# SeanNobel/speech-decoding

Measured on AMD Instinct MI355X. Metric: train segments/sec (Gwilliams2022 208ch x 360, top-10 retrieval acc alongside), higher is better.
Workload: dtype bf16; 1 GPU; Gwilliams2022-shaped MEG: 208 ch x 360 samples, 27 subjects, F=1024, batch 256/GPU, fwd+CLIP loss+top-k+bwd+Adam (BASELINE configs[1]); global_batch=256, seq_len=360, parallelism=dp1

## Files before the change

include/sd_amd.h:

```cpp
#ifndef SD_AMD_H
#define SD_AMD_H
#include <stddef.h>
#include <stdint.h>

#ifdef __cplusplus
extern "C" {
#endif

#define SDA_ABI_VERSION 4
#define SDA_ROW_PAD 16
#define SDA_CH_ALIGN 64

enum { SDA_F32 = 0, SDA_BF16 = 1, SDA_F16 = 2 };

enum { SDA_EPI_GELU = 1,
       SDA_EPI_GLU_BWD = 4,
       SDA_EPI_GLU = 2,
       SDA_CONV_SINGLE_TILE = 4096,
       SDA_CONV_PAIR_TILES = 8192,
       SDA_CONV_ONE_PER_CU = 32768,
       SDA_CONV_FLAT_TILES = 16384,
       SDA_CONV_WIDE_TILES = 524288,
       SDA_CONV_WAVE_PRIO = 1048576,
       SDA_EPI_GELU_BWD = 65536,
// ... 80 lines not shown
                                const float* gamma, const float* beta, int C, float* partial, float* dgamma,
                                float* dbeta, int B, int T, int Cp, int dtype, void* stream);
int sda_reduce_stats(const float* partial, int nrows, float* out0, float* out1, int Cp, void* stream);
int sda_bn_gelu_backward_from_stats(const float* partial, int nrows, const void* dy, const void* x, const float* mean,
                                    const float* rstd, const float* gamma, const float* beta, int C, double count,
                                    float* dgamma, float* dbeta, float* coef, void* dx, int B, int T, int Cp, int dtype,
                                    void* stream);
int sda_bn_gelu_backward_apply(const void* dy, const void* x, const float* mean, const float* rstd,
                               const float* gamma, const float* beta, int C, const float* dgamma,
                               const float* dbeta, double count, float* coef , void* dx,
                               int B, int T, int Cp, int dtype, void* stream);
int sda_bn_gelu_backward_from_stats_dg(const float* partial, int nrows, const void* dy, const void* x, const float* mean,
                                    const float* rstd, const float* gamma, const float* beta, int C, double count,
                                    float* dgamma, float* dbeta, float* coef, void* dx, int B, int T, int Cp, int dtype,
                                    void* stream);
int sda_bn_gelu_backward_apply_dg(const void* dy, const void* x, const float* mean, const float* rstd,
                               const float* gamma, const float* beta, int C, const float* dgamma,
                               const float* dbeta, double count, float* coef , void* dx,
                               int B, int T, int Cp, int dtype, void* stream);

int sda_reduce_scratch_floats(int Cp);

int sda_zero_pad_rows(void* buf, int B, int T, int Cp, int dtype, void* stream);
int sda_fill_zero(void* p, long nbytes, void* stream);
int sda_gather_samples(const void* table, const long* idx, void* dst, int B, long sample_bytes, void* stream);
int sda_scalar_mul(const float* a, const float* b, float* out, int n, void* stream);

int sda_glu_forward(const void* x, void* y, int B, int T, int Ch, int dtype, void* stream);
int sda_glu_backward(const void* x, const void* dy, void* dx, int B, int T, int Ch, int dtype, void* stream);
int sda_gelu_backward(const void* u, const void* dz, void* du, int B, int T, int Cp, int dtype, void* stream);
int sda_reduce_scratch_rows(int B, int T);
int sda_glu_backward_colsum(const void* x, const void* dy, void* dx, float* colsum, float* scratch, int B, int T,
                            int Ch, int dtype, void* stream);
int sda_gelu_backward_colsum(const void* u, const void* dz, void* du, float* colsum, float* scratch, int B, int T,
                             int Cp, int dtype, void* stream);
int sda_glu_backward_colsum_og(const void* out, const void* gate, const void* dy, void* dx, float* colsum, float* scratch,
                               int B, int T, int Ch, int dtype, void* stream);
int sda_colsum(const void* x, float* out, float* scratch , int B, int T,
               int Cp, int dtype, void* stream);

enum { SDA_WGRAD_FLAT_ROWS = 1   };
typedef struct sda_wgrad_args {
  const void* dy;
  const void* x;
  float* g;
  void* out_e;
// ... 25 lines not shown
int sda_sa_softmax_pack(const float* a, int a_pitch, const float* mask, float* W, void* Wp, int D1, int C, int D1p,
                        int Cp, int dtype, void* stream);
int sda_sa_softmax_backward(const float* dWd, int dwd_pitch, const float* W, const float* mask, float* da,
                            int da_pitch, int D1, int C, void* stream);
int sda_sa_weights_backward(const float* dWd, const float* W, const float* mask, const float* cosT,
                            const float* sinT, float* dz, int D1, int K2, int C, int Cp, void* stream);

int sda_clip_logits_stats(const float* S, long s_pitch, const float* ysq, const float* zsq, const float* temp,
                          float* logits, float* row_max, float* row_sum, float* col_lse, float* diag , float* row_lse ,
                          int Bm, int Bn, int col0, void* stream);
int sda_clip_grad(const float* logits, const float* row_lse, const float* col_lse, const float* ysq,
                  const float* zsq, const float* temp, float inv_norm, int col0, void* G, long g_pitch,
                  float* rscale, float* cscale, float* colpart, float* scalars, int Bm, int Bn, int dtype, void* stream);
int sda_clip_grad_y(const float* logits, const float* row_lse, const float* col_lse, const float* zsq,
                    const float* zsq_all, int nz, int col0, void* Gy, long gy_pitch, int seg, int seg_pitch,
                    float* part, int Bm, int Bn, int dtype, void* stream);
int sda_clip_grad_y_finish(const float* part, int nparts, int Bg, const float* ysq, const float* zsq_all, int nz,
                           const float* temp, float inv_norm, int row0, int nrows, float* rscale_y, float* cscale_y,
                           void* stream);
int sda_clip_dz_supported(int Bm, int Bn, long row_elems, int dtype);
int sda_clip_dz(const void* G, long g_pitch, const void* Y, const void* Z, void* out, const float* cscale, const float* rscale,
                const float* out_scale, int Bm, int Bn, long row_elems, int dtype, void* stream);
int sda_clip_ranks(const float* logits, const float* diag, int32_t* cnt, int Bm, int Bn, int col0, void* stream);
int sda_clip_merge_rows(const float* all, int world, int Bg, float* lse, float* diag, void* stream);
int sda_device_count(void);
int sda_stream_create_cumask(const uint32_t* mask, int nwords, void** stream);
int sda_stream_create_priority(int priority, void** stream);
int sda_stream_destroy(void* stream);
int sda_set_cu_limit(int cus);

typedef struct sda_pgemm_args {
  const float* A;
  const float* B;
  void* C;
  int M, N, K, batch;
  long a_i, a_k, a_b;
  long b_k, b_j, b_b;
  long c_i, c_j, c_b;
  int c_dtype;
} sda_pgemm_args;
int sda_param_gemm(const sda_pgemm_args* a, void* stream);
int sda_copy3d(float* dst, long d0, long d1, long d2, const float* src, long s0, long s1, long s2, int n0, int n1, int n2,
               void* stream);
int sda_upload_words(void* dst, const void* src_host, long nwords, void* stream);

int sda_collate_rows(const float* src, float* dst, long rows, int T, int baseline_len, float clamp_lim, int clamp,
// ... 33 lines not shown
```

speech_decoding_amd/csrc/elementwise.hip:

```cpp
#include <math.h>

#include "sd_common.h"

namespace sda {

#ifndef SDA_EW_BWD_PRIO
#define SDA_EW_BWD_PRIO 3
#endif
__device__ __forceinline__ void ew_bwd_prio() {
  if constexpr (SDA_EW_BWD_PRIO > 0) __builtin_amdgcn_s_setprio(SDA_EW_BWD_PRIO);
}

struct RowWalk {
  int r, r1, step, T, b, t;
  __device__ RowWalk(int r0, int r1_, int step_, int T_) : r(r0), r1(r1_), step(step_), T(T_) {
    b = r0 / T_;
    t = r0 - b * T_;
  }
  __device__ bool valid() const { return r < r1; }
  __device__ size_t mem_row() const { return (size_t)b * rows_tp(T) + PAD + t; }
  __device__ void next() {
    r += step; t += step;
    while (t >= T) { t -= T; ++b; }
  }
// ... 858 lines not shown
  for (long i = (long)blockIdx.x * 256 + threadIdx.x; i < pad_vecs + tail_vecs; i += (long)gridDim.x * 256) {
    long v;
    if (i < pad_vecs) { const long b = i / ((long)PAD * row_vec), r = i - b * PAD * row_vec; v = b * Tp * row_vec + r; }
    else v = (long)B * Tp * row_vec + (i - pad_vecs);
    buf[v] = make_uint4(0u, 0u, 0u, 0u);
  }
}
__global__ __launch_bounds__(256) void fill_zero_kernel(uint4* __restrict__ p, long n16, int tail) {
  for (long i = (long)blockIdx.x * 256 + threadIdx.x; i < n16; i += (long)gridDim.x * 256) p[i] = make_uint4(0u, 0u, 0u, 0u);
  if (blockIdx.x == 0 && (int)threadIdx.x < tail) reinterpret_cast<unsigned char*>(p + n16)[threadIdx.x] = 0;
}
__global__ __launch_bounds__(256) void gather_samples_kernel(const uint4* __restrict__ table, const long* __restrict__ idx,
                                                             uint4* __restrict__ dst, long vecs) {
  const uint4* __restrict__ src = table + (size_t)idx[blockIdx.y] * vecs;
  uint4* __restrict__ out = dst + (size_t)blockIdx.y * vecs;
  long i = (long)blockIdx.x * 256 + threadIdx.x;
  const long step = (long)gridDim.x * 256;
  for (; i + 3 * step < vecs; i += 4 * step) {
    const uint4 a = src[i], b = src[i + step], c = src[i + 2 * step], d = src[i + 3 * step];
    out[i] = a; out[i + step] = b; out[i + 2 * step] = c; out[i + 3 * step] = d;
  }
  for (; i < vecs; i += step) out[i] = src[i];
}
__global__ void scalar_mul_kernel(const float* __restrict__ a, const float* __restrict__ b, float* __restrict__ out, int n) {
  const int i = blockIdx.x * blockDim.x + threadIdx.x;
  if (i < n) out[i] = a[i] * b[0];
}
}

extern "C" int sda_zero_pad_rows(void* buf, int B, int T, int Cp, int dtype, void* stream) {
  if (!buf || B < 1 || T < 1 || Cp % 64) { set_error("zero_pad_rows: bad arguments"); return -1; }
  const int row_vec = Cp * (dtype == SDA_F32 ? 4 : 2) / 16;
  const long n = ((long)B * PAD + (rows_alloc(B, T) - (long)B * rows_tp(T))) * row_vec;
  const long blocks = (n + 255) / 256;
  hipLaunchKernelGGL(zero_pad_rows_kernel, dim3((unsigned)(blocks < 1024 ? blocks : 1024)), dim3(256), 0, (hipStream_t)stream,
                     (uint4*)buf, B, rows_tp(T), rows_alloc(B, T), row_vec);
  return check_launch("zero_pad_rows");
}

extern "C" int sda_fill_zero(void* p, long nbytes, void* stream) {
  if (!p || nbytes < 1 || (reinterpret_cast<uintptr_t>(p) & 15)) { set_error("fill_zero: null, empty or unaligned buffer"); return -1; }
  const long n16 = nbytes / 16;
  const long blocks = (n16 + 255) / 256;
  hipLaunchKernelGGL(fill_zero_kernel, dim3((unsigned)(blocks < 1 ? 1 : (blocks > 2048 ? 2048 : blocks))), dim3(256), 0, (hipStream_t)stream,
                     (uint4*)p, n16, (int)(nbytes - n16 * 16));
  return check_launch("fill_zero");
}

extern "C" int sda_gather_samples(const void* table, const long* idx, void* dst, int B, long sample_bytes, void* stream) {
  if (!table || !idx || !dst || B < 1 || sample_bytes < 16 || sample_bytes % 16 || (reinterpret_cast<uintptr_t>(table) & 15) ||
      (reinterpret_cast<uintptr_t>(dst) & 15)) {
    set_error("gather_samples: bad arguments (samples are whole 16-byte vectors)"); return -1;
  }
  const long vecs = sample_bytes / 16;
  long bx = (vecs + 256 * 4 - 1) / (256 * 4);
  const long want = (8L * launch_cus() + B - 1) / B;
  if (bx > want) bx = want;
  if (bx < 1) bx = 1;
  hipLaunchKernelGGL(gather_samples_kernel, dim3((unsigned)bx, (unsigned)B), dim3(256), 0, (hipStream_t)stream,
                     (const uint4*)table, idx, (uint4*)dst, vecs);
// ... 409 lines not shown
```

speech_decoding_amd/csrc/sa_loss.hip:

```cpp
#include "sd_common.h"

namespace sda {

__device__ inline float block_sum(float v, float* sh) {
  v = wave_sum(v);
  __syncthreads();
  if ((threadIdx.x & 63) == 0) sh[threadIdx.x >> 6] = v;
  __syncthreads();
  return sh[0] + sh[1] + sh[2] + sh[3];
}
__device__ inline float block_max(float v, float* sh) {
  v = wave_max(v);
  __syncthreads();
  if ((threadIdx.x & 63) == 0) sh[threadIdx.x >> 6] = v;
  __syncthreads();
  return fmaxf(fmaxf(sh[0], sh[1]), fmaxf(sh[2], sh[3]));
}

constexpr int SA_R = 8;
constexpr int SA_MC = 128;

__global__ __launch_bounds__(256) void sa_fwd_partial_kernel(const float* __restrict__ z, const float* __restrict__ cos_t,
                                                             const float* __restrict__ sin_t, float* __restrict__ part,
                                                             int D1, int K2, int C) {
// ... 258 lines not shown
  pd[threadIdx.x] = dt;
  __syncthreads();
  if (threadIdx.x != 0) return;
  l = 0.0; dt = 0.0;
  for (int k = 0; k < 64; ++k) { l += pl[k]; dt += pd[k]; }
  scalars[0] = (float)(l * (double)inv_norm);
  scalars[1] = (float)dt;
}

__global__ __launch_bounds__(256) void clip_ranks_kernel(const float* __restrict__ logits, const float* __restrict__ diag,
                                                         int32_t* __restrict__ cnt, int Bm, int Bn, int col0) {
  __shared__ float sh[4];
  const int i = blockIdx.x, tid = threadIdx.x;
  const float d = diag[i];
  float c = 0.f;
  for (int j = tid; j < Bn; j += 256) {
    const float l = logits[(size_t)i * Bn + j];
    if (l > d || (l == d && col0 + j < i)) c += 1.f;
  }
  c = block_sum(c, sh);
  if (tid == 0) cnt[i] = (int32_t)(c + 0.5f);
}

}

using namespace sda;

extern "C" int sda_sa_scratch_floats(int D1, int K2, int C) { return ((K2 + SA_MC - 1) / SA_MC) * D1 * C; }

extern "C" int sda_sa_weights_forward(const float* z, const float* cos_t, const float* sin_t, const float* mask, float* W,
                                      void* Wp, float* scratch, int D1, int K2, int C, int D1p, int Cp, int dtype, void* stream) {
  if (!z || !cos_t || !sin_t || !W || !Wp || !scratch || C > 512 || C > Cp || D1 > D1p) { set_error("sa_weights_forward: bad arguments (C <= 512)"); return -1; }
  hipStream_t st = (hipStream_t)stream;
  const int nchunk = (K2 + SA_MC - 1) / SA_MC;
  hipLaunchKernelGGL(sa_fwd_partial_kernel, dim3((D1 + SA_R - 1) / SA_R, nchunk), dim3(256), 0, st, z, cos_t, sin_t, scratch, D1, K2, C);
  if (dtype == SDA_F32)
    hipLaunchKernelGGL(sa_fwd_final_kernel<float>, dim3(D1p), dim3(256), 0, st, scratch, nchunk, C, mask, W, (float*)Wp, D1, C, Cp);
  else if (dtype == SDA_BF16)
    hipLaunchKernelGGL(sa_fwd_final_kernel<uint16_t>, dim3(D1p), dim3(256), 0, st, scratch, nchunk, C, mask, W, (uint16_t*)Wp, D1, C, Cp);
  else if (dtype == SDA_F16)
    hipLaunchKernelGGL(sa_fwd_final_kernel<half_t>, dim3(D1p), dim3(256), 0, st, scratch, nchunk, C, mask, W, (half_t*)Wp, D1, C, Cp);
  else { set_error("sa_weights_forward: unknown dtype"); return -1; }
  return check_launch("sa_weights_forward");
}

extern "C" int sda_sa_softmax_pack(const float* a, int a_pitch, const float* mask, float* W, void* Wp, int D1, int C,
                                   int D1p, int Cp, int dtype, void* stream) {
  if (!a || !W || !Wp || C > 512 || C > Cp || D1 > D1p || a_pitch < C) { set_error("sa_softmax_pack: bad arguments (C <= 512)"); return -1; }
  hipStream_t st = (hipStream_t)stream;
// ... 121 lines not shown
```

speech_decoding_amd/engine.py:

```python
from __future__ import annotations

from dataclasses import dataclass, field
from typing import Dict, List, Optional

import ast
import os

import numpy as np
import torch

from . import lib as L
from . import ops


def block_dilations(k: int):
    return 2 ** ((2 * k) % 5), 2 ** ((2 * k + 1) % 5), 2


@dataclass
class EncoderDims:
    C: int
    S: int
    D1: int
    D2: int
# ... 673 lines not shown
@dataclass
class ClipCtx:
    Bm: int
    Bn: int
    col0: int
    G: torch.Tensor
    rscale: torch.Tensor
    Yt: torch.Tensor
    Zt: torch.Tensor
    row_elems: int
    dtemp: torch.Tensor
    cscale: Optional[torch.Tensor] = None
    logits: Optional[torch.Tensor] = None
    row_lse: Optional[torch.Tensor] = None
    col_lse: Optional[torch.Tensor] = None
    ysq: Optional[torch.Tensor] = None
    zsq: Optional[torch.Tensor] = None
    temp: Optional[torch.Tensor] = None
    inv_norm: float = 0.0


def clip_forward(Yt: torch.Tensor, Zt: torch.Tensor, temp: torch.Tensor, *, Bm: int, Bn: int, T: int, col0: int = 0,
                 reduction: str = "mean", B_global: Optional[int] = None, dist_group=None, want_grad: bool = True,
                 ysq: Optional[torch.Tensor] = None):
    st = clip_block_stats(Yt, Zt, temp, Bm=Bm, Bn=Bn, T=T, col0=col0, ysq=ysq)
    if dist_group is None:
        row_lse, diag = st.row_lse, st.diag
    else:
        from .distributed import merge_row_softmax_stats
        row_lse, diag = merge_row_softmax_stats(st.row_max, st.row_sum, dist_group, diag=st.diag)
    return clip_block_finish(st, row_lse, diag, reduction=reduction, B_global=B_global)


@dataclass
class ClipBlockStats:
    Yt: torch.Tensor
    Zt: torch.Tensor
    temp: torch.Tensor
    Bm: int
    Bn: int
    col0: int
    row_elems: int
    ysq: torch.Tensor
    zsq: torch.Tensor
    logits: torch.Tensor
    row_max: torch.Tensor
    row_sum: torch.Tensor
    col_lse: torch.Tensor
    diag: torch.Tensor
    row_lse: torch.Tensor


def clip_block_stats(Yt, Zt, temp, *, Bm: int, Bn: int, T: int, col0: int = 0, ysq=None) -> ClipBlockStats:
    Fp = Zt.shape[1]
# ... 32 lines not shown
```

speech_decoding_amd/lib.py:

```python
from __future__ import annotations

import ctypes as C
import os

_HERE = os.path.dirname(os.path.abspath(__file__))
LIB_PATH = os.path.join(_HERE, "libsdamd.so")

ABI_VERSION = 4
F32, BF16, F16 = 0, 1, 2
ROW_PAD = 16
CH_ALIGN = 64
EPI_GELU, EPI_GLU, EPI_GLU_BWD = 1, 2, 4
EPI_GELU_BWD, EPI_ROW_SUMSQ, EPI_BN_STORE_DG = 65536, 131072, 262144
CONV_SINGLE_TILE, CONV_PAIR_TILES, CONV_FLAT_TILES, CONV_ONE_PER_CU = 4096, 8192, 16384, 32768
CONV_WAVE_PRIO = 1048576
CONV_WIDE_TILES = 524288
WGRAD_FLAT_ROWS = 1

vp, i32, i64, f32, f64 = C.c_void_p, C.c_int, C.c_long, C.c_float, C.c_double


class ConvArgs(C.Structure):
    _fields_ = [("x", vp), ("w", vp), ("bias", vp), ("res", vp), ("y", vp), ("y_pre", vp), ("widx", vp),
                ("stats", vp), ("partial", vp), ("bn_x", vp), ("bn_coef", vp), ("glu_out", vp), ("glu_gate", vp),
# ... 86 lines not shown
    "sda_sa_scratch_floats": (i32, [i32, i32, i32]),
    "sda_sa_softmax_pack": (i32, [vp, i32, vp, vp, vp, i32, i32, i32, i32, i32, vp]),
    "sda_sa_softmax_backward": (i32, [vp, i32, vp, vp, vp, i32, i32, i32, vp]),
    "sda_sa_weights_backward": (i32, [vp, vp, vp, vp, vp, vp, i32, i32, i32, i32, vp]),
    "sda_clip_logits_stats": (i32, [vp, i64, vp, vp, vp, vp, vp, vp, vp, vp, vp, i32, i32, i32, vp]),
    "sda_clip_grad": (i32, [vp, vp, vp, vp, vp, vp, f32, i32, vp, i64, vp, vp, vp, vp, i32, i32, i32, vp]),
    "sda_clip_grad_y": (i32, [vp, vp, vp, vp, vp, i32, i32, vp, i64, i32, i32, vp, i32, i32, i32, vp]),
    "sda_clip_grad_y_finish": (i32, [vp, i32, i32, vp, vp, i32, vp, f32, i32, i32, vp, vp, vp]),
    "sda_collate_rows": (i32, [vp, vp, i64, i32, i32, f32, i32, vp]),
    "sda_collate_windows": (i32, [vp, vp, vp, i32, i32, i32, i32, f32, i32, vp]),
    "sda_clip_ranks": (i32, [vp, vp, vp, i32, i32, i32, vp]),
    "sda_clip_dz_supported": (i32, [i32, i32, i64, i32]),
    "sda_clip_dz": (i32, [vp, i64, vp, vp, vp, vp, vp, vp, i32, i32, i64, i32, vp]),
    "sda_param_gemm": (i32, [C.POINTER(PgemmArgs), vp]),
    "sda_zero_pad_rows": (i32, [vp, i32, i32, i32, i32, vp]),
    "sda_scalar_mul": (i32, [vp, vp, vp, i32, vp]),
    "sda_fill_zero": (i32, [vp, i64, vp]),
    "sda_gather_samples": (i32, [vp, vp, vp, i32, i64, vp]),
    "sda_clip_merge_rows": (i32, [vp, i32, i32, vp, vp, vp]),
    "sda_copy3d": (i32, [vp, i64, i64, i64, vp, i64, i64, i64, i32, i32, i32, vp]),
    "sda_mse_forward": (i32, [vp, i32, i32, vp, i32, i32, i32, i32, i32, i32, vp, vp, vp]),
    "sda_mse_backward": (i32, [vp, i32, i32, vp, i32, i32, i32, i32, i32, i32, vp, vp, vp, vp]),
    "sda_input_grad": (i32, [vp, i64, vp, vp, i32, i32, i32, i32, i32, i32, i32, vp, i32, vp]),
}
MSE_PARTIALS = 2048

_lib = None


class SdaError(RuntimeError):
    pass


def load():
    global _lib
    if _lib is not None:
        return _lib
    if not os.path.exists(LIB_PATH):
        raise SdaError(
            f"{LIB_PATH} not found: the HIP extension is required (no CPU fallback). "
            "Build it with `python -c 'import __graft_entry__ as g; g.build()'` "
            "or `make -C speech_decoding_amd/csrc`.")
    lib = C.CDLL(LIB_PATH)
    for name, (res, args) in SIGNATURES.items():
        fn = getattr(lib, name)
        fn.restype = res
# ... 24 lines not shown
```

speech_decoding_amd/loss.py:

```python
from __future__ import annotations

from typing import Optional

import torch
import torch.nn as nn

from . import lib as L
from . import ops
from . import engine as E

import weakref

_rank_cache = []


class LossState:

    def __init__(self):
        self.rings = {}
        self.prefetched = []
        self.ring_depth = 2
        self.emulated = {}

    def drain(self):
# ... 170 lines not shown
        Yt, ysq, Bm, col0, Bg, works, slot = gather_speech_rows(Yt_local, B, T, group, async_op=True, state=state, slot=slot)
    state.prefetched.clear()
    state.prefetched.append((weakref.ref(Y), dtype, Yt, ysq, Bm, col0, Bg, works, done, slot))


def _take_prefetched(state: LossState, Y, dtype):
    for wy, dt, Yt, ysq, Bm, col0, Bg, works, done, slot in state.prefetched:
        if wy() is Y and dt == dtype:
            state.prefetched.clear()
            if done is not None:
                torch.cuda.current_stream(Yt.device).wait_event(done)
            for work in works:
                work.wait()
            return Yt, ysq, Bm, col0, Bg, slot
    return None


_RECYCLED = ("CLIPLoss.backward: the packed {what} rows of this forward were recycled by later forwards of the same CLIPLoss "
             "(more than `ring_depth` forwards before this backward); raise loss_func._state.ring_depth or call backward earlier")


class _ClipFn(torch.autograd.Function):
    @staticmethod
    def forward(ctx, module: "CLIPLoss", Y, Z, temp):
        import torch.distributed as dist
        B, F, T = Z.shape
        dtype = Z.dtype if Z.dtype in ops.COMPUTE_DTYPES else torch.float32
        Zt = as_rows(Z, B, F, T, dtype, "y (brain embeddings)")
        group = _dist_group() if module.global_negatives else None
        state = module._state
        want_y = ctx.needs_input_grad[1]
        y_rows = False
        if want_y:
            y_rows = _rows_base(Y, B, F, T, dtype) is not None
            if not y_rows and not Y.is_cuda:
                raise L.SdaError("CLIPLoss: x (speech embeddings) must live on the MI355X device (there is no CPU path)")
            if not y_rows and Y.dtype not in ops.COMPUTE_DTYPES:
                raise L.SdaError(f"CLIPLoss: a speech embedding that requires a gradient must be fp32, bf16 or fp16, got {Y.dtype}")
            if group is not None and dist.get_world_size(group) == 1:
                from .distributed import emulated_world
                if emulated_world() > 1:
                    raise L.SdaError("CLIPLoss: the emulated world (stand-in rows for the other ranks) has no gradient for the "
                                     "speech embeddings; detach x or run real ranks")
        pre = _take_prefetched(state, Y, dtype)
        if pre is not None:
            Yt, ysq, Bm, col0, Bg, slot = pre
        else:
            Yt_local, slot = as_rows(Y, B, F, T, dtype, "x (speech embeddings)", ring_key="loss.Y", state=state, want_slot=True)
            Yt, ysq, Bm, col0, Bg, _, slot = gather_speech_rows(Yt_local, B, T, group, state=state, slot=slot)
        loss, logits, cnt, cctx = E.clip_forward(Yt, Zt, temp.detach(), Bm=Bm, Bn=B, T=T, col0=col0,
                                                 reduction=module.reduction, B_global=Bg, dist_group=group, ysq=ysq)
        ctx.z_gather = None
        if want_y and group is not None:
            Zall, zsq_all, _, _, _, works, zslot = gather_speech_rows(Zt, B, T, group, async_op=True, state=state,
                                                                      ring_key="loss.Zall", sq=cctx.zsq)
            ctx.z_gather = (Zall, zsq_all, works, zslot)
        if group is not None:
            both = torch.cat([cnt.to(torch.float32), loss.reshape(1)])
            dist.all_reduce(both, group=group)
            cnt, loss = both[:-1].round().to(torch.int32), both[-1:]
        ctx.cctx, ctx.shape, ctx.dtype, ctx.group = cctx, (B, F, T), dtype, group
        ctx.set_materialize_grads(False)
        ctx.y_slot = slot
        ctx.z_requires_grad = Z.requires_grad
        ctx.y_requires_grad, ctx.y_rows, ctx.y_dtype = want_y, y_rows, Y.dtype
        _cache_ranks(Y, Z, cnt[col0: col0 + B])
        ctx.mark_non_differentiable(logits)
        return loss.reshape(()), logits

    @staticmethod
    def backward(ctx, dloss, _dlogits):
        c = ctx.cctx
        B, F, T = ctx.shape
        dZ = dY = None
        if dloss is None:
            return None, None, None, None
        scale = dloss.to(torch.float32)
        if (ctx.z_requires_grad or ctx.y_requires_grad) and ctx.y_slot is not None and not ctx.y_slot.valid():
            raise L.SdaError(_RECYCLED.format(what="speech"))
        if ctx.z_requires_grad:
            dZt = ops.new_rows_uninit(B, T, c.Zt.shape[1], ctx.dtype, c.Zt.device)
            E.clip_backward(c, dZt, scale.reshape(1).contiguous())
            dZ = ops.rows_view(dZt, B, F, T)
        if ctx.y_requires_grad:
            dYt = _clip_dy(ctx, scale.reshape(1).contiguous())
            dY = ops.rows_view(dYt, B, F, T) if ctx.y_rows else ops.unpack_rows_typed(dYt, B, F, T, ctx.y_dtype)
        dtemp = ops.scalar_mul(c.dtemp, scale.reshape(1))
        return None, dY, dZ, dtemp


def _clip_dy(ctx, scale: torch.Tensor) -> torch.Tensor:
    c = ctx.cctx
    B, F, T = ctx.shape
    dYt = ops.new_rows_uninit(B, T, c.Yt.shape[1], ctx.dtype, c.Yt.device)
    if ctx.group is None:
        E.clip_backward_y(c, dYt, scale)
        return dYt
    import torch.distributed as dist
    from .distributed import side_group
    world, rank = dist.get_world_size(ctx.group), dist.get_rank(ctx.group)
    Zall, zsq_all, works, zslot = ctx.z_gather
    for work in works:
        work.wait()
    if not zslot.valid():
        raise L.SdaError(_RECYCLED.format(what="brain"))
    Bg, sp = c.Bm, L.pad_channels(B)
    Gy, part = ops.clip_grad_y(c.logits, c.row_lse, c.col_lse, c.zsq, zsq_all, c.col0, ctx.dtype, seg=B, seg_pitch=sp,
                               groups=world)
    Gall = torch.empty((Bg + 1, world * sp), dtype=ctx.dtype, device=Gy.device)
    ops.fill_zero_(Gall[Bg])
    pall = torch.empty((world * part.shape[0], Bg), dtype=torch.float32, device=Gy.device)
# ... 13 lines not shown
        L.load()
        self.reduction = str(args.reduction)
        if self.reduction not in ("mean", "sum"):
            raise ValueError("reduction must be 'mean' or 'sum'")
        self.temp = nn.Parameter(torch.tensor([float(args.init_temperature)]))
        self.global_negatives = True
        self.last_logits: Optional[torch.Tensor] = None
        self._state = LossState()

    def prefetch(self, x: torch.Tensor, compute_dtype=torch.float32):
        prefetch_speech(x, compute_dtype, self.global_negatives, state=self._state)

    def drain(self):
        self._state.drain()

    def release_buffers(self):
        self._state.clear()

    def forward(self, x, y, fast=True, return_logits=False):
        batch_size = x.size(0)
        assert batch_size > 1, "Batch size must be greater than 1."
        if not fast:
            zero = torch.zeros(1, dtype=torch.float32, device=self.temp.device)
            loss, logits = _ClipFn.apply(self, x, y, zero)
            self.last_logits = logits
            return (logits.t(), loss) if return_logits else loss
        loss, logits = _ClipFn.apply(self, x, y, self.temp)
        self.last_logits = logits
        if return_logits:
            return logits, loss
        return loss


@torch.no_grad()
def retrieval_ranks(Y: torch.Tensor, Z: torch.Tensor, global_candidates: bool = True) -> torch.Tensor:
    hit = _cached_ranks(Y, Z)
    if hit is not None:
        return hit
    B, F, T = Z.shape
    dtype = Z.dtype if Z.dtype in ops.COMPUTE_DTYPES else torch.float32
    Zt = as_rows(Z, B, F, T, dtype, "Z")
    Yt = as_rows(Y, B, F, T, dtype, "Y")
    temp = torch.zeros(1, dtype=torch.float32, device=Zt.device)
    group = _dist_group() if global_candidates else None
    Yt, ysq, Bm, col0, Bg, _, _ = gather_speech_rows(Yt, B, T, group)
    _, _, cnt, _ = E.clip_forward(Yt, Zt, temp, Bm=Bm, Bn=B, T=T, col0=col0, B_global=Bg, dist_group=group, ysq=ysq)
    if group is not None:
        import torch.distributed as dist
        dist.all_reduce(cnt, group=group)
    return cnt[col0: col0 + B]
# ... 75 lines not shown
```

speech_decoding_amd/ops.py:

```python
from __future__ import annotations

import ctypes as C
import os
from typing import Optional

import numpy as np
import torch

from . import lib as L

_DT = {torch.float32: L.F32, torch.bfloat16: L.BF16, torch.float16: L.F16}
COMPUTE_DTYPES = tuple(_DT)


def dt_code(dtype: torch.dtype) -> int:
    try:
        return _DT[dtype]
    except KeyError:
        raise L.SdaError(f"unsupported compute dtype {dtype}; use torch.float32, torch.bfloat16 or torch.float16")


def _p(t: Optional[torch.Tensor]):
    return None if t is None else t.data_ptr()

# ... 103 lines not shown
        raise L.SdaError("fill_zero_: a contiguous tensor")
    if t.numel():
        L.check(L.load().sda_fill_zero(t.data_ptr(), t.numel() * t.element_size(), _st()), "fill_zero")
    return t


def gather_samples(table: torch.Tensor, idx: torch.Tensor, B: int, T: int) -> torch.Tensor:
    _need_cuda(table, idx)
    if idx.dtype != torch.int64 or idx.numel() != B:
        raise L.SdaError("gather_samples: idx must hold B int64 indices")
    Cp = table.shape[1]
    out = new_rows_uninit(B, T, Cp, table.dtype, table.device)
    L.check(L.load().sda_gather_samples(_p(table), _p(idx), _p(out), B, L.rows_tp(T) * Cp * table.element_size(), _st()), "gather_samples")
    return out


def clip_merge_rows(allp: torch.Tensor):
    world, k, Bg = allp.shape
    if k != 3 or allp.dtype != torch.float32 or not allp.is_contiguous():
        raise L.SdaError("clip_merge_rows: a contiguous fp32 (world, 3, B_global) table")
    out = torch.empty((2, Bg), dtype=torch.float32, device=allp.device)
    L.check(L.load().sda_clip_merge_rows(_p(allp), world, Bg, _p(out[0]), _p(out[1]), _st()), "clip_merge_rows")
    return out[0], out[1]


def scalar_mul(a: torch.Tensor, b: torch.Tensor) -> torch.Tensor:
    out = torch.empty_like(a)
    L.check(L.load().sda_scalar_mul(_p(a), _p(b), _p(out), a.numel(), _st()), "scalar_mul")
    return out


def rows_view(buf: torch.Tensor, B: int, C: int, T: int) -> torch.Tensor:
    Tp, Cp = L.rows_tp(T), buf.shape[1]
    return buf.as_strided((B, C, T), (Tp * Cp, 1, Cp), L.ROW_PAD * Cp)


def pack_rows(src: torch.Tensor, dst: torch.Tensor, ones_channel: Optional[int] = None):
    _need_cuda(src, dst)
    B, Cc, T = src.shape
    src = src.contiguous().float()
    if ones_channel is None:
        L.check(L.load().sda_pack_rows(_p(src), _p(dst), B, Cc, T, dst.shape[1], dt_code(dst.dtype), _st()), "pack_rows")
    else:
        L.check(L.load().sda_pack_rows_ones(_p(src), _p(dst), B, Cc, T, dst.shape[1], ones_channel, dt_code(dst.dtype), _st()),
                "pack_rows_ones")

# ... 302 lines not shown
        cin, cout = alg_dims if alg_dims is not None else (x.shape[1], y.shape[1])
        e0, e1 = torch.cuda.Event(enable_timing=True), torch.cuda.Event(enable_timing=True)
        e0.record()
        L.check(L.load().sda_conv_gemm(C.byref(a), _st()), "conv_gemm")
        e1.record()
        TIMER.records.append((("conv_gemm", str(x.dtype).replace("torch.", ""), conv_tile_co(Cout_p, KS, stats is not None), KS),
                              2.0 * B * T * KS * cin * cout, e0, e1))
        return y
    L.check(L.load().sda_conv_gemm(C.byref(a), _st()), "conv_gemm")
    return y


def n_t_tiles(T: int) -> int:
    return (T + 127) // 128


def conv_stats_rows(B: int, T: int, KS: int, Cout_p: int, flags: int = 0) -> int:
    return L.load().sda_conv_stats_rows(B, T, KS, Cout_p, flags)


SIM_GEMM_TILES256 = os.environ.get("SDA_SIM_GEMM", "1") != "0"


def matmul_nt_splitk(xm: torch.Tensor, wm: torch.Tensor, M: int, N: int, K: int, pitch: int) -> torch.Tensor:
    Np = L.pad_channels(N)
    if SIM_GEMM_TILES256 and K <= pitch:
        ks = L.load().sda_sim_gemm_ksplit(M, N, K, dt_code(xm.dtype))
        if ks > 0:
            partial = torch.empty((ks, M, Np), dtype=torch.float32, device=xm.device)
            L.check(L.load().sda_sim_gemm(_p(xm), _p(wm), _p(partial), M, N, Np, K, pitch, ks, dt_code(xm.dtype), _st()), "sim_gemm")
            if ks == 1:
                return partial[0]
            out = torch.empty((M, Np), dtype=torch.float32, device=xm.device)
            L.check(L.load().sda_reduce_slabs(_p(partial), _p(out), ks, M * Np, _st()), "reduce_slabs")
            return out
    slab = 32 if xm.dtype == torch.float32 else 64
    nslab = K // slab
    tile_co = 160 if Np % 160 == 0 else (128 if Np % 128 == 0 else 64)
    tiles = ((M + 127) // 128) * (Np // tile_co)
    ksplit = max(1, min(nslab, (512 + tiles - 1) // tiles))
    if nslab <= 64:
        ksplit = min(ksplit, 16)
    partial = torch.empty((ksplit, M, Np), dtype=torch.float32, device=xm.device)
    a = L.ConvArgs()
    a.x, a.w, a.bias, a.res, a.y, a.y_pre, a.widx, a.stats = _p(xm), _p(wm), None, None, None, None, None, None
    a.partial = _p(partial)
    a.B, a.T, a.Cin_p, a.Cout_p, a.KS, a.dil = 1, M, K, Np, 1, 0
    a.x_pitch, a.w_pitch, a.x_row0, a.x_sample_rows, a.x_rows_limit = pitch, pitch, 0, 0, M
    a.w_rows_limit, a.ksplit, a.flags, a.dtype = N, ksplit, 0, dt_code(xm.dtype)
    L.check(L.load().sda_conv_gemm(C.byref(a), _st()), "conv_gemm(split-K)")
    if ksplit == 1:
        return partial[0]
    out = torch.empty((M, Np), dtype=torch.float32, device=xm.device)
    L.check(L.load().sda_reduce_slabs(_p(partial), _p(out), ksplit, M * Np, _st()), "reduce_slabs")
    return out


def bn_finalize(partial, ntiles, count, gamma, beta, running_mean, running_var, Cp, training, eps=1e-5, momentum=0.1,
                want_bwd_coef=False, batches_tracked=None):
    if batches_tracked is not None and (batches_tracked.dtype != torch.int64 or not batches_tracked.is_cuda):
        raise L.SdaError("bn_finalize: batches_tracked must be an int64 device tensor")
    dev = gamma.device
    buf = torch.empty((8 if want_bwd_coef else 4, Cp), dtype=torch.float32, device=dev)
    mean, rstd, scale, shift = buf[0], buf[1], buf[2], buf[3]
    coef = buf[4:] if want_bwd_coef else None
    L.check(L.load().sda_bn_finalize(_p(partial), ntiles, float(count), _p(gamma), _p(beta), eps, momentum,
                                     _p(running_mean), _p(running_var), _p(mean), _p(rstd), _p(scale), _p(shift),
                                     _p(coef), gamma.numel(), Cp, int(training), _p(batches_tracked), _st()), "bn_finalize")
    return (mean, rstd, scale, shift, coef) if want_bwd_coef else (mean, rstd, scale, shift)


def bn_gelu_forward(x, y, scale, shift, B, T):
    L.check(L.load().sda_bn_gelu_forward(_p(x), _p(y), _p(scale), _p(shift), B, T, x.shape[1], dt_code(x.dtype), _st()),
# ... 233 lines not shown
    st3 = torch.empty((3, Bm), dtype=torch.float32, device=dev)
    row_max, row_sum, diag = st3[0], st3[1], st3[2]
    col_lse = torch.empty(Bn, dtype=torch.float32, device=dev)
    row_lse = torch.empty(Bm, dtype=torch.float32, device=dev)
    L.check(L.load().sda_clip_logits_stats(_p(S), S.shape[1], _p(ysq), _p(zsq), _p(temp), _p(logits), _p(row_max), _p(row_sum),
                                           _p(col_lse), _p(diag), _p(row_lse), Bm, Bn, col0, _st()), "clip_logits_stats")
    return logits, row_max, row_sum, col_lse, diag, row_lse


def clip_grad(logits, row_lse, col_lse, ysq, zsq, temp, inv_norm, col0, dtype):
    Bm, Bn = logits.shape
    dev = logits.device
    G = torch.empty((Bm + 1, L.pad_channels(Bn)), dtype=dtype, device=dev)
    rscale = torch.empty(Bn, dtype=torch.float32, device=dev)
    cscale = torch.empty(Bn, dtype=torch.float32, device=dev)
    colpart = torch.empty(2 * Bn, dtype=torch.float32, device=dev)
    scalars = torch.empty(2, dtype=torch.float32, device=dev)
    L.check(L.load().sda_clip_grad(_p(logits), _p(row_lse), _p(col_lse), _p(ysq), _p(zsq), _p(temp), float(inv_norm), col0,
                                   _p(G), G.shape[1], _p(rscale), _p(cscale), _p(colpart), _p(scalars), Bm, Bn, dt_code(dtype), _st()),
            "clip_grad")
    return G, rscale, cscale, scalars


def clip_grad_y(logits, row_lse, col_lse, zsq, zsq_all, col0, dtype, *, seg=None, seg_pitch=None, groups=1):
    Bm, Bn = logits.shape
    seg = Bm if seg is None else seg
    seg_pitch = L.pad_channels(seg) if seg_pitch is None else seg_pitch
    dev = logits.device
    Gy = torch.empty((Bn + 1, groups * seg_pitch), dtype=dtype, device=dev)
    part = torch.empty(((Bn + 63) // 64, Bm), dtype=torch.float32, device=dev)
    L.check(L.load().sda_clip_grad_y(_p(logits), _p(row_lse), _p(col_lse), _p(zsq), _p(zsq_all), zsq_all.numel(), col0, _p(Gy),
                                     Gy.shape[1], seg, seg_pitch, _p(part), Bm, Bn, dt_code(dtype), _st()), "clip_grad_y")
    return Gy, part


def clip_grad_y_finish(part, ysq, zsq_all, temp, inv_norm, row0, nrows):
    nparts, Bg = part.shape
    rscale = torch.empty(nrows, dtype=torch.float32, device=part.device)
    cscale = torch.empty(nrows, dtype=torch.float32, device=part.device)
    L.check(L.load().sda_clip_grad_y_finish(_p(part), nparts, Bg, _p(ysq), _p(zsq_all), zsq_all.numel(), _p(temp), float(inv_norm),
                                            row0, nrows, _p(rscale), _p(cscale), _st()), "clip_grad_y_finish")
    return rscale, cscale


def clip_ranks(logits, diag, col0):
    Bm, Bn = logits.shape
# ... 76 lines not shown
```

Before: 38070 segments/s.

## Fuse CLIP split-K reduction, logits stats, ranks and grad into two kernels

The single-GPU CLIP forward path now keeps the split-K similarity partials unreduced. A row kernel sums the slabs while computing logits, row softmax stats and rank counts, and a column kernel computes column LSE, the gradient matrix, scales and the final loss scalars, using a last-block atomic reduction. The backward pass also folds the dtemp scalar multiply into the zero-padding kernel for dZ. The aim is fewer small kernel launches in the loss section. The cost is a grid-wide atomic counter and a limit of 256 rows for the fused path.

```diff
diff --git a/include/sd_amd.h b/include/sd_amd.h
--- a/include/sd_amd.h
+++ b/include/sd_amd.h
@@ -126,6 +126,8 @@
 int sda_reduce_scratch_floats(int Cp);
 
 int sda_zero_pad_rows(void* buf, int B, int T, int Cp, int dtype, void* stream);
+int sda_zero_pad_rows_scaled(void* buf, int B, int T, int Cp, int dtype, const float* a, const float* b, float* out, int n,
+                             void* stream);
 int sda_fill_zero(void* p, long nbytes, void* stream);
 int sda_gather_samples(const void* table, const long* idx, void* dst, int B, long sample_bytes, void* stream);
 int sda_scalar_mul(const float* a, const float* b, float* out, int n, void* stream);
@@ -197,6 +199,11 @@
 int sda_clip_dz(const void* G, long g_pitch, const void* Y, const void* Z, void* out, const float* cscale, const float* rscale,
                 const float* out_scale, int Bm, int Bn, long row_elems, int dtype, void* stream);
 int sda_clip_ranks(const float* logits, const float* diag, int32_t* cnt, int Bm, int Bn, int col0, void* stream);
+int sda_clip_stats_fused_max_rows(void);
+int sda_clip_stats_fused(const float* slabs, int nslabs, long slab_elems, long s_pitch, const float* ysq, const float* zsq,
+                         const float* temp, const float* dloss, float inv_norm, float* logits, float* row_max, float* row_sum,
+                         float* row_lse, float* col_lse, float* diag, void* G, long g_pitch, float* rscale, float* cscale,
+                         float* colpart, float* scalars, int32_t* cnt, unsigned* counter, int B, int dtype, void* stream);
 int sda_clip_merge_rows(const float* all, int world, int Bg, float* lse, float* diag, void* stream);
 int sda_device_count(void);
 int sda_stream_create_cumask(const uint32_t* mask, int nwords, void** stream);
diff --git a/speech_decoding_amd/csrc/elementwise.hip b/speech_decoding_amd/csrc/elementwise.hip
--- a/speech_decoding_amd/csrc/elementwise.hip
+++ b/speech_decoding_amd/csrc/elementwise.hip
@@ -904,6 +904,19 @@
   }
   for (; i < vecs; i += step) out[i] = src[i];
 }
+__global__ __launch_bounds__(256) void zero_pad_rows_scaled_kernel(uint4* __restrict__ buf, int B, int Tp, long rows_alloc, int row_vec,
+                                                                   const float* __restrict__ a, const float* __restrict__ b,
+                                                                   float* __restrict__ out, int n) {
+  if (blockIdx.x == 0)
+    for (int i = threadIdx.x; i < n; i += 256) out[i] = a[i] * b[0];
+  const long pad_vecs = (long)B * PAD * row_vec, tail_vecs = (rows_alloc - (long)B * Tp) * row_vec;
+  for (long i = (long)blockIdx.x * 256 + threadIdx.x; i < pad_vecs + tail_vecs; i += (long)gridDim.x * 256) {
+    long v;
+    if (i < pad_vecs) { const long bb = i / ((long)PAD * row_vec), r = i - bb * PAD * row_vec; v = bb * Tp * row_vec + r; }
+    else v = (long)B * Tp * row_vec + (i - pad_vecs);
+    buf[v] = make_uint4(0u, 0u, 0u, 0u);
+  }
+}
 __global__ void scalar_mul_kernel(const float* __restrict__ a, const float* __restrict__ b, float* __restrict__ out, int n) {
   const int i = blockIdx.x * blockDim.x + threadIdx.x;
   if (i < n) out[i] = a[i] * b[0];
@@ -918,6 +931,17 @@
   hipLaunchKernelGGL(zero_pad_rows_kernel, dim3((unsigned)(blocks < 1024 ? blocks : 1024)), dim3(256), 0, (hipStream_t)stream,
                      (uint4*)buf, B, rows_tp(T), rows_alloc(B, T), row_vec);
   return check_launch("zero_pad_rows");
+}
+
+extern "C" int sda_zero_pad_rows_scaled(void* buf, int B, int T, int Cp, int dtype, const float* a, const float* b, float* out, int n,
+                                        void* stream) {
+  if (!buf || B < 1 || T < 1 || Cp % 64 || !a || !b || !out || n < 1) { set_error("zero_pad_rows_scaled: bad arguments"); return -1; }
+  const int row_vec = Cp * (dtype == SDA_F32 ? 4 : 2) / 16;
+  const long nv = ((long)B * PAD + (rows_alloc(B, T) - (long)B * rows_tp(T))) * row_vec;
+  const long blocks = (nv + 255) / 256;
+  hipLaunchKernelGGL(zero_pad_rows_scaled_kernel, dim3((unsigned)(blocks < 1024 ? blocks : 1024)), dim3(256), 0, (hipStream_t)stream,
+                     (uint4*)buf, B, rows_tp(T), rows_alloc(B, T), row_vec, a, b, out, n);
+  return check_launch("zero_pad_rows_scaled");
 }
 
 extern "C" int sda_fill_zero(void* p, long nbytes, void* stream) {
diff --git a/speech_decoding_amd/csrc/sa_loss.hip b/speech_decoding_amd/csrc/sa_loss.hip
--- a/speech_decoding_amd/csrc/sa_loss.hip
+++ b/speech_decoding_amd/csrc/sa_loss.hip
@@ -304,9 +304,145 @@
   if (tid == 0) cnt[i] = (int32_t)(c + 0.5f);
 }
 
+__global__ __launch_bounds__(256) void clip_stats_rows_kernel(const float* __restrict__ slabs, int nslabs, long slab_elems,
+                                                              long s_pitch, const float* __restrict__ ysq,
+                                                              const float* __restrict__ zsq, const float* __restrict__ temp,
+                                                              float* __restrict__ logits, float* __restrict__ row_max,
+                                                              float* __restrict__ row_sum, float* __restrict__ diag,
+                                                              float* __restrict__ row_lse, int32_t* __restrict__ cnt,
+                                                              unsigned* __restrict__ counter, int B) {
+  __shared__ float sh[4];
+  __shared__ float dsh;
+  const int i = blockIdx.x, tid = threadIdx.x;
+  const bool valid = tid < B;
+  if (i == 0 && tid == 0) *counter = 0u;
+  const float alpha = expf(temp[0]);
+  const float ri = alpha / sqrtf(ysq[i]);
+  float l = -INFINITY;
+  if (valid) {
+    const float* __restrict__ src = slabs + (size_t)i * s_pitch + tid;
+    float s = 0.f;
+    int k = 0;
+    for (; k + 8 <= nslabs; k += 8) {
+      float v[8];
+#pragma unroll
+      for (int j = 0; j < 8; ++j) v[j] = src[(size_t)(k + j) * slab_elems];
+#pragma unroll
+      for (int j = 0; j < 8; ++j) s += v[j];
+    }
+    for (; k < nslabs; ++k) s += src[(size_t)k * slab_elems];
+    l = s * ri / sqrtf(zsq[tid]);
+    logits[(size_t)i * B + tid] = l;
+    if (tid == i) { diag[i] = l; dsh = l; }
+  }
+  const float mx = block_max(l, sh);
+  const float sum = block_sum(valid ? expf(l - mx) : 0.f, sh);
+  if (tid == 0) { row_max[i] = mx; row_sum[i] = sum; row_lse[i] = mx + logf(sum); }
+  const float d = dsh;
+  float c = 0.f;
+  if (valid && (l > d || (l == d && tid < i))) c += 1.f;
+  c = block_sum(c, sh);
+  if (tid == 0) cnt[i] = (int32_t)(c + 0.5f);
+}
+
+template <typename E>
+__global__ __launch_bounds__(256) void clip_stats_cols_kernel(const float* __restrict__ logits, const float* __restrict__ row_lse,
+                                                              const float* __restrict__ ysq, const float* __restrict__ zsq,
+                                                              const float* __restrict__ temp, const float* __restrict__ dloss,
+                                                              float inv_norm, float* __restrict__ col_lse, E* __restrict__ G,
+                                                              long g_pitch, float* __restrict__ rscale, float* __restrict__ cscale,
+                                                              float* colpart, float* __restrict__ scalars, unsigned* counter, int B) {
+  __shared__ float sh[4];
+  __shared__ double pl[64], pd[64];
+  __shared__ int last;
+  const int j = blockIdx.x, tid = threadIdx.x;
+  const bool valid = tid < B;
+  if (tid == 0) Elem<E>::st(G + (size_t)B * g_pitch + j, 0.f);
+  if (j >= B) {
+    if (valid) Elem<E>::st(G + (size_t)tid * g_pitch + j, 0.f);
+  } else {
+    const float l = valid ? logits[(size_t)tid * B + j] : -INFINITY;
+    const float mx = block_max(l, sh);
+    const float sum = block_sum(valid ? expf(l - mx) : 0.f, sh);
+    const float cl = mx + logf(sum);
+    const float ymax = sqrtf(block_max(valid ? fmaxf(0.f, ysq[tid]) : 0.f, sh));
+    const float alpha = expf(temp[0]);
+    float dl = 0.f;
+    if (valid) {
+      float d = expf(l - row_lse[tid]) + expf(l - cl);
+      if (tid == j) d -= 2.f;
+      dl += d * l;
+      Elem<E>::st(G + (size_t)tid * g_pitch + j, d * (ymax / sqrtf(ysq[tid])));
+    }
+    dl = block_sum(dl, sh) * inv_norm;
+    if (tid == 0) {
+      const float ljj = logits[(size_t)j * B + j];
+      col_lse[j] = cl;
+      rscale[j] = dl / zsq[j];
+      cscale[j] = inv_norm * alpha / (ymax * sqrtf(zsq[j]));
+      colpart[j * 2 + 0] = (row_lse[j] - ljj) + (cl - ljj);
+      colpart[j * 2 + 1] = dl;
+    }
+  }
+  if (tid == 0) {
+    __threadfence();
+    const unsigned t = __hip_atomic_fetch_add(counter, 1u, __ATOMIC_ACQ_REL, __HIP_MEMORY_SCOPE_AGENT);
+    last = (t == gridDim.x - 1);
+  }
+  __syncthreads();
+  if (!last) return;
+  __threadfence();
+  if (tid < 64) {
+    double ls = 0.0, dt = 0.0;
+    for (int k = tid; k < B; k += 64) {
+      ls += (double)__hip_atomic_load(colpart + k * 2, __ATOMIC_RELAXED, __HIP_MEMORY_SCOPE_AGENT);
+      dt += (double)__hip_atomic_load(colpart + k * 2 + 1, __ATOMIC_RELAXED, __HIP_MEMORY_SCOPE_AGENT);
+    }
+    pl[tid] = ls;
+    pd[tid] = dt;
+  }
+  __syncthreads();
+  if (tid != 0) return;
+  double ls = 0.0, dt = 0.0;
+  for (int k = 0; k < 64; ++k) { ls += pl[k]; dt += pd[k]; }
+  scalars[0] = (float)(ls * (double)inv_norm);
+  scalars[1] = (float)dt;
+  if (dloss) scalars[2] = (float)dt * dloss[0];
+}
+
 }
 
 using namespace sda;
+
+extern "C" int sda_clip_stats_fused_max_rows(void) { return 256; }
+
+extern "C" int sda_clip_stats_fused(const float* slabs, int nslabs, long slab_elems, long s_pitch, const float* ysq,
+                                    const float* zsq, const float* temp, const float* dloss, float inv_norm, float* logits,
+                                    float* row_max, float* row_sum, float* row_lse, float* col_lse, float* diag, void* G,
+                                    long g_pitch, float* rscale, float* cscale, float* colpart, float* scalars, int32_t* cnt,
+                                    unsigned* counter, int B, int dtype, void* stream) {
+  if (!slabs || !ysq || !zsq || !temp || !logits || !row_max || !row_sum || !row_lse || !col_lse || !diag || !G || !rscale ||
+      !cscale || !colpart || !scalars || !cnt || !counter) { set_error("clip_stats_fused: null argument"); return -1; }
+  if (B < 1 || B > 256 || nslabs < 1 || s_pitch < B || slab_elems < (long)(B - 1) * s_pitch + B || g_pitch < B || g_pitch > 65535) {
+    set_error("clip_stats_fused: 1 <= B <= 256 rows and columns, slabs of at least B rows of s_pitch >= B floats, g_pitch >= B");
+    return -1;
+  }
+  hipStream_t st = (hipStream_t)stream;
+  hipLaunchKernelGGL(clip_stats_rows_kernel, dim3(B), dim3(256), 0, st, slabs, nslabs, slab_elems, s_pitch, ysq, zsq, temp, logits,
+                     row_max, row_sum, diag, row_lse, cnt, counter, B);
+  const dim3 grid((unsigned)g_pitch);
+  if (dtype == SDA_F32)
+    hipLaunchKernelGGL(clip_stats_cols_kernel<float>, grid, dim3(256), 0, st, logits, row_lse, ysq, zsq, temp, dloss, inv_norm, col_lse,
+                       (float*)G, g_pitch, rscale, cscale, colpart, scalars, counter, B);
+  else if (dtype == SDA_BF16)
+    hipLaunchKernelGGL(clip_stats_cols_kernel<uint16_t>, grid, dim3(256), 0, st, logits, row_lse, ysq, zsq, temp, dloss, inv_norm, col_lse,
+                       (uint16_t*)G, g_pitch, rscale, cscale, colpart, scalars, counter, B);
+  else if (dtype == SDA_F16)
+    hipLaunchKernelGGL(clip_stats_cols_kernel<half_t>, grid, dim3(256), 0, st, logits, row_lse, ysq, zsq, temp, dloss, inv_norm, col_lse,
+                       (half_t*)G, g_pitch, rscale, cscale, colpart, scalars, counter, B);
+  else { set_error("clip_stats_fused: unknown dtype"); return -1; }
+  return check_launch("clip_stats_fused");
+}
 
 extern "C" int sda_sa_scratch_floats(int D1, int K2, int C) { return ((K2 + SA_MC - 1) / SA_MC) * D1 * C; }
 
diff --git a/speech_decoding_amd/engine.py b/speech_decoding_amd/engine.py
--- a/speech_decoding_amd/engine.py
+++ b/speech_decoding_amd/engine.py
@@ -719,7 +719,9 @@
 
 def clip_forward(Yt: torch.Tensor, Zt: torch.Tensor, temp: torch.Tensor, *, Bm: int, Bn: int, T: int, col0: int = 0,
                  reduction: str = "mean", B_global: Optional[int] = None, dist_group=None, want_grad: bool = True,
-                 ysq: Optional[torch.Tensor] = None):
+                 ysq: Optional[torch.Tensor] = None, fused: bool = False):
+    if fused and dist_group is None and Bm == Bn and col0 == 0 and Bm <= ops.clip_stats_fused_max_rows():
+        return _clip_forward_fused(Yt, Zt, temp, B=Bm, T=T, reduction=reduction, B_global=B_global, ysq=ysq)
     st = clip_block_stats(Yt, Zt, temp, Bm=Bm, Bn=Bn, T=T, col0=col0, ysq=ysq)
     if dist_group is None:
         row_lse, diag = st.row_lse, st.diag
@@ -727,6 +729,23 @@
         from .distributed import merge_row_softmax_stats
         row_lse, diag = merge_row_softmax_stats(st.row_max, st.row_sum, dist_group, diag=st.diag)
     return clip_block_finish(st, row_lse, diag, reduction=reduction, B_global=B_global)
+
+
+def _clip_forward_fused(Yt, Zt, temp, *, B: int, T: int, reduction: str, B_global: Optional[int], ysq):
+    row_elems = L.rows_tp(T) * Zt.shape[1]
+    if ysq is None:
+        ysq = ops.rows_sumsq(Yt, B, row_elems, row_elems)
+    zsq = ops.ROW_NORMS.get(Zt, B)
+    if zsq is None:
+        zsq = ops.rows_sumsq(Zt, B, row_elems, row_elems)
+    slabs = ops.matmul_nt_splitk(Yt, Zt, B, B, row_elems, row_elems, reduce=False)
+    Bg = B_global if B_global is not None else B
+    inv_norm = 1.0 / (2.0 * Bg) if reduction == "mean" else 0.5
+    logits, _, _, col_lse, _, row_lse, G, rscale, cscale, scalars, cnt = ops.clip_stats_fused(slabs, ysq, zsq, temp, inv_norm,
+                                                                                              Yt.dtype, B)
+    ctx = ClipCtx(Bm=B, Bn=B, col0=0, G=G, rscale=rscale, Yt=Yt, Zt=Zt, row_elems=row_elems, dtemp=scalars[1:2],
+                  cscale=cscale, logits=logits, row_lse=row_lse, col_lse=col_lse, ysq=ysq, zsq=zsq, temp=temp, inv_norm=inv_norm)
+    return scalars[0:1], logits, cnt, ctx
 
 
 @dataclass
diff --git a/speech_decoding_amd/lib.py b/speech_decoding_amd/lib.py
--- a/speech_decoding_amd/lib.py
+++ b/speech_decoding_amd/lib.py
@@ -132,6 +132,10 @@
     "sda_mse_forward": (i32, [vp, i32, i32, vp, i32, i32, i32, i32, i32, i32, vp, vp, vp]),
     "sda_mse_backward": (i32, [vp, i32, i32, vp, i32, i32, i32, i32, i32, i32, vp, vp, vp, vp]),
     "sda_input_grad": (i32, [vp, i64, vp, vp, i32, i32, i32, i32, i32, i32, i32, vp, i32, vp]),
+    "sda_clip_stats_fused_max_rows": (i32, []),
+    "sda_clip_stats_fused": (i32, [vp, i32, i64, i64, vp, vp, vp, vp, f32, vp, vp, vp, vp, vp, vp, vp, i64, vp, vp, vp, vp, vp, vp,
+                                   i32, i32, vp]),
+    "sda_zero_pad_rows_scaled": (i32, [vp, i32, i32, i32, i32, vp, vp, vp, i32, vp]),
 }
 MSE_PARTIALS = 2048
 
diff --git a/speech_decoding_amd/loss.py b/speech_decoding_amd/loss.py
--- a/speech_decoding_amd/loss.py
+++ b/speech_decoding_amd/loss.py
@@ -216,7 +216,7 @@
 
 class _ClipFn(torch.autograd.Function):
     @staticmethod
-    def forward(ctx, module: "CLIPLoss", Y, Z, temp):
+    def forward(ctx, module: "CLIPLoss", Y, Z, temp, fast):
         import torch.distributed as dist
         B, F, T = Z.shape
         dtype = Z.dtype if Z.dtype in ops.COMPUTE_DTYPES else torch.float32
@@ -243,7 +243,8 @@
             Yt_local, slot = as_rows(Y, B, F, T, dtype, "x (speech embeddings)", ring_key="loss.Y", state=state, want_slot=True)
             Yt, ysq, Bm, col0, Bg, _, slot = gather_speech_rows(Yt_local, B, T, group, state=state, slot=slot)
         loss, logits, cnt, cctx = E.clip_forward(Yt, Zt, temp.detach(), Bm=Bm, Bn=B, T=T, col0=col0,
-                                                 reduction=module.reduction, B_global=Bg, dist_group=group, ysq=ysq)
+                                                 reduction=module.reduction, B_global=Bg, dist_group=group, ysq=ysq,
+                                                 fused=fast and group is None and not want_y)
         ctx.z_gather = None
         if want_y and group is not None:
             Zall, zsq_all, _, _, _, works, zslot = gather_speech_rows(Zt, B, T, group, async_op=True, state=state,
@@ -268,19 +269,21 @@
         B, F, T = ctx.shape
         dZ = dY = None
         if dloss is None:
-            return None, None, None, None
+            return None, None, None, None, None
         scale = dloss.to(torch.float32)
         if (ctx.z_requires_grad or ctx.y_requires_grad) and ctx.y_slot is not None and not ctx.y_slot.valid():
             raise L.SdaError(_RECYCLED.format(what="speech"))
         if ctx.z_requires_grad:
-            dZt = ops.new_rows_uninit(B, T, c.Zt.shape[1], ctx.dtype, c.Zt.device)
+            dZt, dtemp = ops.zero_pad_rows_scaled(torch.empty((L.rows_alloc(B, T), c.Zt.shape[1]), dtype=ctx.dtype, device=c.Zt.device),
+                                                  B, T, c.dtemp, scale.reshape(1))
             E.clip_backward(c, dZt, scale.reshape(1).contiguous())
             dZ = ops.rows_view(dZt, B, F, T)
         if ctx.y_requires_grad:
             dYt = _clip_dy(ctx, scale.reshape(1).contiguous())
             dY = ops.rows_view(dYt, B, F, T) if ctx.y_rows else ops.unpack_rows_typed(dYt, B, F, T, ctx.y_dtype)
-        dtemp = ops.scalar_mul(c.dtemp, scale.reshape(1))
-        return None, dY, dZ, dtemp
+        if not ctx.z_requires_grad:
+            dtemp = ops.scalar_mul(c.dtemp, scale.reshape(1))
+        return None, dY, dZ, dtemp, None
 
 
 def _clip_dy(ctx, scale: torch.Tensor) -> torch.Tensor:
@@ -340,10 +343,10 @@
         assert batch_size > 1, "Batch size must be greater than 1."
         if not fast:
             zero = torch.zeros(1, dtype=torch.float32, device=self.temp.device)
-            loss, logits = _ClipFn.apply(self, x, y, zero)
+            loss, logits = _ClipFn.apply(self, x, y, zero, False)
             self.last_logits = logits
             return (logits.t(), loss) if return_logits else loss
-        loss, logits = _ClipFn.apply(self, x, y, self.temp)
+        loss, logits = _ClipFn.apply(self, x, y, self.temp, True)
         self.last_logits = logits
         if return_logits:
             return logits, loss
diff --git a/speech_decoding_amd/ops.py b/speech_decoding_amd/ops.py
--- a/speech_decoding_amd/ops.py
+++ b/speech_decoding_amd/ops.py
@@ -149,6 +149,13 @@
     out = torch.empty((2, Bg), dtype=torch.float32, device=allp.device)
     L.check(L.load().sda_clip_merge_rows(_p(allp), world, Bg, _p(out[0]), _p(out[1]), _st()), "clip_merge_rows")
     return out[0], out[1]
+
+
+def zero_pad_rows_scaled(buf: torch.Tensor, B: int, T: int, a: torch.Tensor, b: torch.Tensor):
+    out = torch.empty_like(a)
+    L.check(L.load().sda_zero_pad_rows_scaled(_p(buf), B, T, buf.shape[1], dt_code(buf.dtype), _p(a), _p(b), _p(out), a.numel(), _st()),
+            "zero_pad_rows_scaled")
+    return buf, out
 
 
 def scalar_mul(a: torch.Tensor, b: torch.Tensor) -> torch.Tensor:
@@ -497,13 +504,15 @@
 SIM_GEMM_TILES256 = os.environ.get("SDA_SIM_GEMM", "1") != "0"
 
 
-def matmul_nt_splitk(xm: torch.Tensor, wm: torch.Tensor, M: int, N: int, K: int, pitch: int) -> torch.Tensor:
+def matmul_nt_splitk(xm: torch.Tensor, wm: torch.Tensor, M: int, N: int, K: int, pitch: int, reduce: bool = True) -> torch.Tensor:
     Np = L.pad_channels(N)
     if SIM_GEMM_TILES256 and K <= pitch:
         ks = L.load().sda_sim_gemm_ksplit(M, N, K, dt_code(xm.dtype))
         if ks > 0:
             partial = torch.empty((ks, M, Np), dtype=torch.float32, device=xm.device)
             L.check(L.load().sda_sim_gemm(_p(xm), _p(wm), _p(partial), M, N, Np, K, pitch, ks, dt_code(xm.dtype), _st()), "sim_gemm")
+            if not reduce:
+                return partial
             if ks == 1:
                 return partial[0]
             out = torch.empty((M, Np), dtype=torch.float32, device=xm.device)
@@ -524,6 +533,8 @@
     a.x_pitch, a.w_pitch, a.x_row0, a.x_sample_rows, a.x_rows_limit = pitch, pitch, 0, 0, M
     a.w_rows_limit, a.ksplit, a.flags, a.dtype = N, ksplit, 0, dt_code(xm.dtype)
     L.check(L.load().sda_conv_gemm(C.byref(a), _st()), "conv_gemm(split-K)")
+    if not reduce:
+        return partial
     if ksplit == 1:
         return partial[0]
     out = torch.empty((M, Np), dtype=torch.float32, device=xm.device)
@@ -803,6 +814,32 @@
     return G, rscale, cscale, scalars
 
 
+def clip_stats_fused_max_rows() -> int:
+    return L.load().sda_clip_stats_fused_max_rows()
+
+
+def clip_stats_fused(slabs, ysq, zsq, temp, inv_norm, dtype, B, dloss=None):
+    if slabs.dim() != 3 or slabs.dtype != torch.float32 or not slabs.is_contiguous() or slabs.shape[1] < B or slabs.shape[2] < B:
+        raise L.SdaError("clip_stats_fused: contiguous fp32 slabs (ks, >= B, >= B)")
+    dev = slabs.device
+    logits = torch.empty((B, B), dtype=torch.float32, device=dev)
+    st3 = torch.empty((3, B), dtype=torch.float32, device=dev)
+    row_max, row_sum, diag = st3[0], st3[1], st3[2]
+    lse = torch.empty((2, B), dtype=torch.float32, device=dev)
+    row_lse, col_lse = lse[0], lse[1]
+    G = torch.empty((B + 1, L.pad_channels(B)), dtype=dtype, device=dev)
+    fac = torch.empty((4, B), dtype=torch.float32, device=dev)
+    rscale, cscale, colpart = fac[0], fac[1], fac[2:]
+    scalars = torch.empty(3, dtype=torch.float32, device=dev)
+    cnt = torch.empty(B, dtype=torch.int32, device=dev)
+    counter = torch.empty(1, dtype=torch.int32, device=dev)
+    L.check(L.load().sda_clip_stats_fused(_p(slabs), slabs.shape[0], slabs.stride(0), slabs.stride(1), _p(ysq), _p(zsq), _p(temp),
+                                          _p(dloss), float(inv_norm), _p(logits), _p(row_max), _p(row_sum), _p(row_lse), _p(col_lse),
+                                          _p(diag), _p(G), G.shape[1], _p(rscale), _p(cscale), _p(colpart), _p(scalars), _p(cnt),
+                                          _p(counter), B, dt_code(dtype), _st()), "clip_stats_fused")
+    return logits, row_max, row_sum, col_lse, diag, row_lse, G, rscale, cscale, scalars, cnt
+
+
 def clip_grad_y(logits, row_lse, col_lse, zsq, zsq_all, col0, dtype, *, seg=None, seg_pitch=None, groups=1):
     Bm, Bn = logits.shape
     seg = Bm if seg is None else seg
```

Result: no change. 38330 segments/s (median of 5 runs) (+0.7%).
